# KKKSQJ/DeepLearning

Measured on NVIDIA H100. Metric: images/sec (ResNet-50 training step), higher is better.
Workload: dtype bf16

## Files before the change

### deeplearning_b200/csrc/abi_conv.cu

```cuda
#include <string.h>
#include "../../include/b200cls.h"
#include "conv_gemm.cuh"
#include "conv1x1_stream.cuh"
#include "conv_tap64.cuh"
#include "host_utils.h"
#include "wgrad_gemm.cuh"

using namespace b200;

namespace {

constexpr uint32_t kFwdDescLbo = 16, kFwdDescSbo = 1024;
constexpr uint32_t kWgDescLbo = 8192, kWgDescSbo = 1024, kWgDescKstep = 2048;

struct Box3 {
  int b1, b2, b3;
};

Box3 choose_box(long long d1, long long d2, long long d3, int P) {
  Box3 best{P, 1, 1};
  double best_cost = -1;
  for (int b1 = 1; b1 <= P; b1 <<= 1) {
    for (int b2 = 1; b1 * b2 <= P; b2 <<= 1) {
      const int b3 = P / (b1 * b2);
      if (b1 > 256 || b2 > 256 || b3 > 256) continue;
      const double c1 = double((d1 + b1 - 1) / b1) * b1, c2 = double((d2 + b2 - 1) / b2) * b2,
                   c3 = double((d3 + b3 - 1) / b3) * b3;
      const double cost = c1 * c2 * c3;
      if (best_cost < 0 || cost < best_cost - 0.5 ||
          (cost < best_cost + 0.5 && (b1 > best.b1 || (b1 == best.b1 && b2 > best.b2)))) {
        best_cost = cost;
        best = Box3{b1, b2, b3};
      }
    }
  }
  return best;
}
// ... 186 lines not shown
  if (p.residual) f |= p.res_f32 ? kEpiResF32 : kEpiResBf16;
  if (p.has_aux_out) f |= kEpiAux;
  if (p.out_f32) f |= kEpiOutF32;
  if (p.out_direct) f |= kEpiDirect;
  if (p.stats) f |= kEpiStats;
  if (p.rowscale) f |= kEpiRowscale;
  if (p.affine) f = (f & ~(kEpiBias | kEpiColscale)) | kEpiAffine;
  if (p.mask_in) f |= p.bn_scale ? kEpiBnMask : kEpiMask;
  if (p.bn_scale) f &= ~kEpiStats;
  return f;
}

#define B200_EPI_LIST(X)                                                                                  \
  X(kEpiStats)                                              \
  X(0)                                                      \
  X(kEpiResBf16)                                            \
  X(kEpiBias)                                               \
  X(kEpiBias | kEpiResF32 | kEpiOutF32)                     \
  X(kEpiBias | kEpiColscale | kEpiResF32 | kEpiOutF32)      \
  X(kEpiBias | (2 << kEpiActShift) | kEpiAux)               \
  X(3 << kEpiActShift)                                      \
  X((3 << kEpiActShift) | kEpiStats)                        \
  X(kEpiOutF32)                                             \
  X(kEpiBias | kEpiOutF32)                                  \
  X(kEpiAffine | kEpiResBf16 | (1 << kEpiActShift))        \
  X(kEpiAffine | (1 << kEpiActShift))                      \
  X(kEpiAffine)                                            \
  X(kEpiMask | kEpiResBf16 | kEpiStats)                    \
  X(kEpiBnMask)                                            \
  X(kEpiBnMask | kEpiBias)                                 \
  X(kEpiBias | (1 << kEpiActShift))                        \
  X(kEpiBias | kEpiStats)

bool tap64_ok(const ConvGemmParams& p) {
  const int f = epilogue_flags(p);
  return p.N == 64 && p.n_tiles == 1 && p.k_per_tap == 64 && p.k_blocks_per_tap == 1 && !p.var_taps && !p.chan_window &&
         p.num_taps >= 2 && p.num_taps <= 9 && (f == 0 || f == kEpiStats) && p.dim1 % p.box1 == 0 && p.dim2 % p.box2 == 0 &&
         p.dim3 % p.box3 == 0;
}
template <bool kStats>
int launch_tap64(const ConvGemmParams& q, int grid, cudaStream_t st) {
  static bool configured = false;
  if (!configured) {
    B200_CHECK_CUDA(cudaFuncSetAttribute(conv_tap64_kernel<kStats>, cudaFuncAttributeMaxDynamicSharedMemorySize, kTap64SmemBytes));
    configured = true;
  }
  B200_CHECK_CUDA(launch_pdl(conv_tap64_kernel<kStats>, dim3(grid), dim3(384), kTap64SmemBytes, st, q));
  B200_LAUNCHED();
  return OK;
}

template <int BLOCK_N>
int launch_conv_gemm(const ConvGemmParams& p, cudaStream_t st) {
  const int tiles = p.tiles1 * p.tiles2 * p.tiles3 * p.n_tiles;
  const int grid = conv_grid(tiles, p.n_tiles, p.stats != nullptr);
  B200_REQUIRE(grid > 0, "conv_gemm: %d channel blocks exceed the SM count (BN statistics need grid %% n_tiles == 0)", p.n_tiles);
  ConvGemmParams q = p;
  q.desc_lbo = kFwdDescLbo;
  q.desc_sbo = kFwdDescSbo;
  if constexpr (BLOCK_N == 64) {
    if (tap64_ok(p)) return p.stats != nullptr ? launch_tap64<true>(q, grid, st) : launch_tap64<false>(q, grid, st);
  }
  switch (epilogue_flags(p)) {
#define B200_EPI_CASE(F) \
  case (F):              \
    return launch_conv_gemm_epi<BLOCK_N, (F)>(q, grid, st);
    B200_EPI_LIST(B200_EPI_CASE)
#undef B200_EPI_CASE
    default:
      return launch_conv_gemm_epi<BLOCK_N, kEpiGeneric>(q, grid, st);
  }
}


bool stream_ok(long long pixels, int K, int N) {
  return (K == 64 || K == 128 || K == 256) && N % 256 == 0 && pixels % 128 == 0 && pixels / 128 < (1LL << 30);
}
int stream_grid(long long pixels, int N) {
  const int n_tiles = N / 256;
  const long long items = pixels / 128 * n_tiles;
  int grid = items < device_sm_count() ? static_cast<int>(items) : device_sm_count();
  return grid / n_tiles * n_tiles;
}

template <int KB, int MODE>
int launch_stream(const StreamParams& q, int grid, cudaStream_t st) {
  using Cfg = StreamCfg<KB, MODE>;
  static bool configured = false;
  if (!configured) {
    B200_CHECK_CUDA(cudaFuncSetAttribute(conv1x1_stream_kernel<KB, MODE>, cudaFuncAttributeMaxDynamicSharedMemorySize,
                                         Cfg::SMEM_BYTES));
    configured = true;
  }
  B200_CHECK_CUDA(launch_pdl(conv1x1_stream_kernel<KB, MODE>, dim3(grid), dim3(Cfg::THREADS), Cfg::SMEM_BYTES, st, q));
// ... 211 lines not shown
  B200_REQUIRE(bn_scale == nullptr || (Cout % 64 == 0 && bias == nullptr && stats == nullptr && out_f32 == nullptr && act <= 1 && !y_f32),
               "conv2d_fwd + folded BN: Cout=%d must be a multiple of 64, no bias / statistics / fp32 output", Cout);
  cudaStream_t st = static_cast<cudaStream_t>(stream);
  const int Ho = out_dim(H, ksize, stride), Wo = out_dim(W, ksize, stride);
  ConvGemmParams p;
  memset(&p, 0, sizeof(p));
  int rc;
  View dv = act_view(y, B, Ho, Wo, Cout, ksize == 1 && stride == 1);
  if (out_f32 != nullptr) dv.base = nullptr;
  if ((rc = setup_output(p, dv, Cout, y_f32, nullptr))) return rc;
  const int BN = Cg ? 64 : block_n_for(Cout);
  p.n_tiles = (Cout + BN - 1) / BN;
  p.chan_window = Cg ? 1 : 0;
  p.k_per_tap = Cg ? 64 : Cin;
  p.k_blocks_per_tap = Cg ? 1 : (Cin + 63) / 64;
  p.num_taps = ksize * ksize;
  if ((rc = encode_taps(p, p.a_maps, x, B, H, W, Cin, ksize, stride, box_of(p)))) return rc;
  for (int t = 0; t < p.num_taps; ++t) p.tap_w[t] = static_cast<int8_t>(t);
  if ((rc = encode_matrix(&p.b_map, w, static_cast<long long>(p.num_taps) * p.k_per_tap, Cout, BN))) return rc;
  p.stats = stats;
  p.bias = bias;
  p.act = act;
  p.residual = residual;
  p.rs1 = static_cast<long long>(dv.strides[1]);
  p.rs2 = static_cast<long long>(dv.strides[2]);
  p.rs3 = static_cast<long long>(dv.strides[3]);
  p.out_direct = out_f32;
  p.ld_out = ld_out;
  if (bn_scale != nullptr) {
    p.affine = 1;
    p.colscale = bn_scale;
    p.bias = bn_shift;
  }
  return Cg ? launch_conv_gemm<64>(p, st) : dispatch_conv_gemm(p, Cout, st);
}

int b200_conv2d_fwd(const void* x, const void* w, void* y, int B, int H, int W, int Cin, int Cout, int ksize, int stride,
                    float* stats, const float* bias, int act, const void* residual, float* out_f32, long long ld_out,
                    const float* bn_scale, const float* bn_shift, void* stream) {
  return conv_fwd(x, w, y, B, H, W, Cin, Cout, ksize, stride, stats, bias, act, residual, out_f32, ld_out, bn_scale, bn_shift,
                  0, 0, stream);
}

int b200_conv2d_fwd_f32(const void* x, const void* w, float* y, int B, int H, int W, int Cin, int Cout, int ksize,
                        int stride, const float* bias, void* stream) {
  return conv_fwd(x, w, y, B, H, W, Cin, Cout, ksize, stride, nullptr, bias, 0, nullptr, nullptr, 0, nullptr, nullptr, 1, 0,
                  stream);
}

static int conv_dgrad(const void* dy, const void* wd, void* dx, int B, int H, int W, int Cin, int Cout, int ksize,
                      int stride, const void* residual, const b200_bn_mask_t* bn_mask, int Cg, void* stream) {
  B200_REQUIRE(ksize == 1 || ksize == 3 || (ksize == 2 && stride == 2), "conv2d_dgrad: ksize %d / stride %d unsupported", ksize, stride);
  B200_REQUIRE(stride == 1 || stride == 2, "conv2d_dgrad: stride %d unsupported", stride);
  B200_REQUIRE(Cin % 8 == 0 && Cout % 8 == 0, "conv2d_dgrad: Cin=%d / Cout=%d must be multiples of 8", Cin, Cout);
  B200_REQUIRE(bn_mask == nullptr || (stride == 1 && Cin % 64 == 0 && bn_mask_complete(bn_mask)),
               "conv2d_dgrad: the fused BatchNorm-backward reduce needs stride 1, Cin %% 64 == 0 and every bn_mask field "
               "(Cin=%d, stride=%d)", Cin, stride);
  cudaStream_t st = static_cast<cudaStream_t>(stream);
  const int Ho = out_dim(H, ksize, stride), Wo = out_dim(W, ksize, stride);
  const bool flat = (ksize == 1 && stride == 1);
  const int BN = Cg ? 64 : block_n_for(Cin);
  const int k_per_tap = Cg ? 64 : Cout;
  int rc;
  CUtensorMap b_map;
  if ((rc = encode_matrix(&b_map, wd, static_cast<long long>(ksize * ksize) * k_per_tap, Cin, BN))) return rc;
  const int nphase = (stride == 2 && ksize >= 2) ? 2 : 1;
// ... 19 lines not shown
        for (int kh = 0; kh < 3; ++kh)
          for (int kw = 0; kw < 3; ++kw) {
            p.tap_map[nt] = 0;
            p.tap_o1[nt] = static_cast<int8_t>(1 - kw);
            p.tap_o2[nt] = static_cast<int8_t>(1 - kh);
            p.tap_w[nt] = static_cast<int8_t>(kh * 3 + kw);
            ++nt;
          }
      } else if (ksize == 2) {
        p.tap_map[0] = 0, p.tap_o1[0] = 0, p.tap_o2[0] = 0;
        p.tap_w[0] = static_cast<int8_t>(ph * 2 + pw);
        nt = 1;
      } else {
        for (int kh = 0; kh < 3; ++kh) {
          if (((ph + 1 - kh) & 1) != 0) continue;
          for (int kw = 0; kw < 3; ++kw) {
            if (((pw + 1 - kw) & 1) != 0) continue;
            p.tap_map[nt] = 0;
            p.tap_o1[nt] = static_cast<int8_t>((pw + 1 - kw) / 2);
            p.tap_o2[nt] = static_cast<int8_t>((ph + 1 - kh) / 2);
            p.tap_w[nt] = static_cast<int8_t>(kh * 3 + kw);
            ++nt;
          }
        }
      }
      p.num_taps = nt;
      if (residual != nullptr) {
        p.residual = static_cast<const char*>(residual) + (static_cast<const char*>(dv.base) - static_cast<const char*>(dx));
        p.rs1 = static_cast<long long>(dv.strides[1]);
        p.rs2 = static_cast<long long>(dv.strides[2]);
        p.rs3 = static_cast<long long>(dv.strides[3]);
      }
      if (bn_mask != nullptr) set_bn_mask(p, bn_mask, dv);
      if ((rc = Cg ? launch_conv_gemm<64>(p, st) : dispatch_conv_gemm(p, Cin, st))) return rc;
    }
  }
  return OK;
}

int b200_conv2d_dgrad(const void* dy, const void* wd, void* dx, int B, int H, int W, int Cin, int Cout, int ksize,
                      int stride, const void* residual, const b200_bn_mask_t* bn_mask, void* stream) {
  return conv_dgrad(dy, wd, dx, B, H, W, Cin, Cout, ksize, stride, residual, bn_mask, 0, stream);
}

int b200_gemm_ex(const b200_view_t* a, const b200_view_t* out, const b200_gemm_args_t* g, void* stream) {
  B200_REQUIRE(a != nullptr && out != nullptr && g != nullptr && g->w != nullptr, "gemm_ex: null argument");
  B200_REQUIRE(g->N % 8 == 0 && g->K % 8 == 0, "gemm_ex: N=%d / K=%d must be multiples of 8", g->N, g->K);
  for (int i = 0; i < 3; ++i)
    B200_REQUIRE(a->dim[i] == out->dim[i] && a->dim[i] > 0, "gemm_ex: a/out pixel extents differ in dim %d", i);
  B200_REQUIRE(!(g->aux_out != nullptr && g->out_f32), "gemm_ex: aux_out needs a bf16 primary output");
  B200_REQUIRE(!(g->stats != nullptr && g->out_f32), "gemm_ex: stats need a bf16 output");
  auto to_view = [](const b200_view_t* v, int C) {
    View r;
    r.base = v->base;
    r.dims[0] = C;
    r.strides[0] = 1;
    for (int i = 0; i < 3; ++i) {
      r.dims[i + 1] = static_cast<uint64_t>(v->dim[i]);
      r.strides[i + 1] = static_cast<uint64_t>(v->stride[i]);
    }
    return r;
  };
  ConvGemmParams p;
  memset(&p, 0, sizeof(p));
  int rc;
  View dv = to_view(out, g->N);
// ... 56 lines not shown
  if (pl.block_ng == 64)
    rc = launch_wgrad<64>(p, st);
  else if (pl.block_ng == 128)
    rc = launch_wgrad<128>(p, st);
  else if (pl.block_ng == 192)
    rc = launch_wgrad<192>(p, st);
  else
    rc = launch_wgrad<256>(p, st);
  if (rc) return rc;
  if ((rc = launch_wgrad_reduce(p.partial, dw, pl.splits, Cout, Cin, pl.taps, accumulate, st, bias_partial, bias_out))) return rc;
  B200_LAUNCHED();
  return OK;
}

int b200_stem_s2d_conv_fwd(const void* z, const void* w, void* y, float* stats, int B, int Ho, int Wo, void* stream) {
  B200_REQUIRE(B > 0 && Ho > 0 && Wo > 0, "stem_s2d_conv_fwd: empty output");
  cudaStream_t st = static_cast<cudaStream_t>(stream);
  const int Cout = 64;
  ConvGemmParams p;
  memset(&p, 0, sizeof(p));
  int rc;
  if ((rc = setup_output(p, make_view(y, B, Ho, Wo, Cout, 1, 0, 0), Cout, 0, nullptr))) return rc;
  const Box3 bx = box_of(p);
  p.k_per_tap = 64;
  p.k_blocks_per_tap = 1;
  p.num_taps = 4;
  if ((rc = encode_view(&p.a_maps[0], stem_s2d_view(z, B, Ho, Wo), bx))) return rc;
  for (int i = 1; i < 4; ++i) p.a_maps[i] = p.a_maps[0];
  for (int ky = 0; ky < 4; ++ky) {
    p.tap_map[ky] = 0, p.tap_o1[ky] = 0, p.tap_o2[ky] = static_cast<int8_t>(ky), p.tap_w[ky] = static_cast<int8_t>(ky);
  }
  if ((rc = encode_matrix(&p.b_map, w, 256, Cout, 64))) return rc;
  p.stats = stats;
  return dispatch_conv_gemm(p, Cout, st);
}

size_t b200_stem_s2d_conv_wgrad_workspace_bytes(int B, int Ho, int Wo) {
  return wgrad_bytes(plan_wgrad_geom(Wo, Ho, B, 64, 64, 4), 64, 64);
}

int b200_stem_s2d_conv_wgrad(const void* dy, const void* z, float* g, void* workspace, size_t workspace_bytes, int B, int Ho,
                             int Wo, void* stream) {
  cudaStream_t st = static_cast<cudaStream_t>(stream);
  const int Cout = 64, Cin = 64, taps = 4;
  const WgradPlan pl = plan_wgrad_geom(Wo, Ho, B, Cin, Cout, taps);
  const size_t need = wgrad_bytes(pl, Cout, Cin);
  B200_REQUIRE(workspace != nullptr && workspace_bytes >= need, "stem_s2d_conv_wgrad: workspace too small (%zu < %zu)",
               workspace_bytes, need);
  WgradParams p = wgrad_params(pl, Cout, Cin, workspace);
  int rc;
  if ((rc = encode_view(&p.dy_map, make_view(dy, B, Ho, Wo, Cout, 1, 0, 0), pl.box))) return rc;
  if ((rc = encode_view(&p.x_maps[0], stem_s2d_view(z, B, Ho, Wo), pl.box))) return rc;
  for (int i = 1; i < 4; ++i) p.x_maps[i] = p.x_maps[0];
  for (int ky = 0; ky < 4; ++ky) p.tap_map[ky] = 0, p.tap_o1[ky] = 0, p.tap_o2[ky] = static_cast<int8_t>(ky);
  if ((rc = launch_wgrad<256>(p, st))) return rc;
  if ((rc = launch_wgrad_reduce(p.partial, g, pl.splits, Cout, Cin, taps, 0, st))) return rc;
  B200_LAUNCHED();
  return OK;
}


int b200_conv1x1_bn_act_fwd(const void* x, const void* w, const float* scale, const float* shift, const void* residual,
                            void* y, long long pixels, int Cin, int Cout, int relu, void* stream) {
  B200_REQUIRE(pixels > 0 && Cin % 64 == 0 && Cout % 64 == 0, "conv1x1_bn_act_fwd: Cin=%d / Cout=%d must be multiples of 64", Cin, Cout);
  B200_REQUIRE(scale != nullptr && shift != nullptr && residual != nullptr && relu == 1,
               "conv1x1_bn_act_fwd: implemented for relu(bn(conv) + residual)");
// ... 162 lines not shown
```

### deeplearning_b200/csrc/conv_gemm.cuh

```cuda
#pragma once
#include <cstdio>
#include "common.cuh"

namespace b200 {

constexpr int kMaxTaps = 16;

struct alignas(64) ConvGemmParams {
  CUtensorMap a_maps[4];
  CUtensorMap b_map;
  CUtensorMap d_map;
  CUtensorMap aux_map;
  int num_taps;
  int k_per_tap;
  int k_blocks_per_tap;
  int tiles1, tiles2, tiles3;
  int box1, box2, box3;
  int dim1, dim2, dim3;
  int qoff1[4], qoff2[4], qoff3[4];
  int n_tiles;
  int N;
  int8_t tap_map[kMaxTaps];
  int8_t tap_o1[kMaxTaps];
  int8_t tap_o2[kMaxTaps];
  int8_t tap_w[kMaxTaps];
  float* stats;
  const float* bias;
  const float* colscale;
  int act;
  int out_f32;
  int res_f32;
  int has_aux_out;
  const void* residual;
  long long rs1, rs2, rs3;
  const __nv_bfloat16* aux_in;
  long long as1, as2, as3;
  uint32_t desc_lbo, desc_sbo;
  float* out_direct;
  long long ld_out;
  const float* rowscale;
  int rows_per_sample;
  int var_taps;
  int kb_total;
  int16_t tap_kb[kMaxTaps];
  int32_t tap_k0[kMaxTaps];
  const __nv_bfloat16* mask_in;
  long long ms1, ms2, ms3;
  int affine;
  const float* bn_scale;
  const float* bn_shift;
  int chan_window;
};

template <int BLOCK_N>
struct ConvGemmCfg {
  static constexpr int BLOCK_M = 128;
  static constexpr int BLOCK_K = 64;
  static constexpr int A_BYTES = BLOCK_M * BLOCK_K * 2;
  static constexpr int B_BYTES = BLOCK_N * BLOCK_K * 2;
  static constexpr int STAGES = BLOCK_N == 128 ? 4 : 5;
  static constexpr int STAGE_BYTES = A_BYTES + B_BYTES;
  static constexpr int EPI_WARPS = 4;
  static constexpr int SLAB_BYTES = 32 * 128;
  static constexpr int STAGING_BYTES = EPI_WARPS * 2 * SLAB_BYTES;
  static constexpr int IMG_BYTES = BLOCK_M * BLOCK_N * 4;
  static constexpr int IMGS = BLOCK_N == 128 ? 1 : 2;
  static constexpr int BAR_BYTES = 256;
  static constexpr int SMEM_BYTES = STAGES * STAGE_BYTES + STAGING_BYTES + IMGS * IMG_BYTES + BAR_BYTES + 1024;
  static constexpr int THREADS = 512;
  static_assert(SMEM_BYTES <= 227 * 1024, "shared memory of one H100 block");
  static_assert(2 * STAGES + 2 * IMGS <= BAR_BYTES / 8, "mbarriers");
};

__device__ __forceinline__ void gelu_parts(float x, float& tail, float& e) {
  const float az = fabsf(x) * 0.70710678118654752f;
  float t;
  asm("rcp.approx.ftz.f32 %0, %1;" : "=f"(t) : "f"(fmaf(0.3275911f, az, 1.0f)));
  float poly = fmaf(1.061405429f, t, -1.453152027f);
  poly = fmaf(poly, t, 1.421413741f);
  poly = fmaf(poly, t, -0.284496736f);
  poly = fmaf(poly, t, 0.254829592f);
  asm("ex2.approx.ftz.f32 %0, %1;" : "=f"(e) : "f"(-1.4426950408889634f * az * az));
  tail = 0.5f * poly * t * e;
}
__device__ __forceinline__ float gelu_erf(float x) {
  float tail, e;
  gelu_parts(x, tail, e);
  return x * (x >= 0.f ? 1.0f - tail : tail);
}
__device__ __forceinline__ float gelu_erf_grad(float x) {
  float tail, e;
  gelu_parts(x, tail, e);
  const float cdf = x >= 0.f ? 1.0f - tail : tail;
  return fmaf(x * 0.3989422804014327f, e, cdf);
}

__device__ __forceinline__ void gelu_parts2(float x0, float x1, uint64_t& cdf, uint64_t& e) {
  const uint64_t az = f2_pack(fabsf(x0) * 0.70710678118654752f, fabsf(x1) * 0.70710678118654752f);
  float d0, d1, t0, t1, g0, g1, e0, e1, h0, h1;
  f2_unpack(f2_fma(f2_bcast(0.3275911f), az, f2_bcast(1.0f)), d0, d1);
  asm("rcp.approx.ftz.f32 %0, %1;" : "=f"(t0) : "f"(d0));
  asm("rcp.approx.ftz.f32 %0, %1;" : "=f"(t1) : "f"(d1));
  const uint64_t t = f2_pack(t0, t1);
  uint64_t poly = f2_fma(f2_bcast(1.061405429f), t, f2_bcast(-1.453152027f));
// ... 15 lines not shown
__device__ __forceinline__ void gelu_erf_val_grad2(float& x0, float& x1, float& g0, float& g1) {
  uint64_t cdf, e;
  gelu_parts2(x0, x1, cdf, e);
  const uint64_t x = f2_pack(x0, x1);
  f2_unpack(f2_fma(f2_mul(x, f2_bcast(0.3989422804014327f)), e, cdf), g0, g1);
  f2_unpack(f2_mul(x, cdf), x0, x1);
}

#ifdef CONV_PROFILE
#define CPROF_DECL(N) long long cp_t[N] = {}; long long cp_0 = clock64(), cp_1;
#define CPROF_TICK(i) { cp_1 = clock64(); cp_t[i] += cp_1 - cp_0; cp_0 = cp_1; }
#else
#define CPROF_DECL(N)
#define CPROF_TICK(i)
#endif

template <int S>
__device__ __forceinline__ void butterfly_step(float (&px)[32], int lane) {
  const bool up = (lane & S) != 0;
#pragma unroll
  for (int i = 0; i < S; ++i) {
    const float send = up ? px[i] : px[i + S];
    const float keep = up ? px[i + S] : px[i];
    px[i] = keep + __shfl_xor_sync(0xffffffffu, send, S);
  }
}

constexpr int kEpiGeneric = -1;
constexpr int kEpiBias = 1, kEpiColscale = 2, kEpiActShift = 2 , kEpiResBf16 = 16, kEpiResF32 = 32,
              kEpiAux = 64, kEpiOutF32 = 128, kEpiDirect = 256, kEpiStats = 512,
              kEpiRowscale = 1024 ,
              kEpiAffine = 2048, kEpiMask = 4096, kEpiBnMask = 8192;

template <int BLOCK_N, int EPI = kEpiGeneric>
__global__ void __launch_bounds__(512, 1) conv_gemm_kernel(const __grid_constant__ ConvGemmParams p) {
  static_assert(BLOCK_N == 64 || BLOCK_N == 128, "64- or 128-column tiles");
  using Cfg = ConvGemmCfg<BLOCK_N>;
  constexpr int STAGES = Cfg::STAGES;
  constexpr int IMGS = Cfg::IMGS;
  extern __shared__ uint8_t smem_raw[];
  uint8_t* smem = reinterpret_cast<uint8_t*>((reinterpret_cast<uintptr_t>(smem_raw) + 1023) & ~uintptr_t(1023));
  uint8_t* stage_base = smem;
  uint8_t* staging = smem + STAGES * Cfg::STAGE_BYTES;
  uint8_t* img = staging + Cfg::STAGING_BYTES;
  uint64_t* bars = reinterpret_cast<uint64_t*>(img + IMGS * Cfg::IMG_BYTES);
  uint64_t* full_bar = bars;
  uint64_t* empty_bar = bars + STAGES;
  uint64_t* img_full = bars + 2 * STAGES;
  uint64_t* img_empty = bars + 2 * STAGES + IMGS;

  const int warp_idx = threadIdx.x >> 5;
  const int lane = threadIdx.x & 31;
  const int m_tiles = p.tiles1 * p.tiles2 * p.tiles3;
  const int num_tiles = m_tiles * p.n_tiles;
  const int num_kb = p.var_taps ? p.kb_total : p.num_taps * p.k_blocks_per_tap;

  if (warp_idx == 0 && lane == 0) {
    for (int i = 0; i < 4; ++i) tma_prefetch_desc(&p.a_maps[i]);
    tma_prefetch_desc(&p.b_map);
    tma_prefetch_desc(&p.d_map);
    for (int i = 0; i < STAGES; ++i) {
      mbar_init(&full_bar[i], 1);
      mbar_init(&empty_bar[i], 2);
    }
    for (int i = 0; i < IMGS; ++i) {
      mbar_init(&img_full[i], 8);
      mbar_init(&img_empty[i], Cfg::EPI_WARPS);
    }
    fence_mbar_init();
  }
  __syncthreads();
  pdl_wait();

  if (warp_idx < 4) {
    setmaxnreg_dec<40>();
    if (warp_idx == 0 && lane == 0) {
      int stage = 0;
      uint32_t phase = 0;
      CPROF_DECL(2)
      for (int tile = blockIdx.x; tile < num_tiles; tile += gridDim.x) {
        const int n_tile = tile % p.n_tiles;
        const int m_tile = tile / p.n_tiles;
        const int t1 = m_tile % p.tiles1;
        const int t2 = (m_tile / p.tiles1) % p.tiles2;
        const int t3 = m_tile / (p.tiles1 * p.tiles2);
        const int c1 = t1 * p.box1, c2 = t2 * p.box2, c3 = t3 * p.box3;
        int tap = 0, cb = 0;
        int kb_in_tap = p.var_taps ? p.tap_kb[0] : p.k_blocks_per_tap;
        for (int kb = 0; kb < num_kb; ++kb, ++cb) {
          if (cb == kb_in_tap) {
            cb = 0;
            ++tap;
            if (p.var_taps) kb_in_tap = p.tap_kb[tap];
          }
          const int wk = p.var_taps ? p.tap_k0[tap] + cb * 64 : p.tap_w[tap] * p.k_per_tap + cb * 64;
          CPROF_TICK(1)
          mbar_wait_backoff(&empty_bar[stage], phase ^ 1);
          CPROF_TICK(0)
          uint8_t* a_dst = stage_base + stage * Cfg::STAGE_BYTES;
          uint8_t* b_dst = a_dst + Cfg::A_BYTES;
          mbar_expect_tx(&full_bar[stage], Cfg::STAGE_BYTES);
          tma_load_4d(a_dst, &p.a_maps[p.tap_map[tap]], &full_bar[stage], p.chan_window ? n_tile * BLOCK_N : cb * 64, c1 + p.tap_o1[tap],
                      c2 + p.tap_o2[tap], c3);
          tma_load_2d(b_dst, &p.b_map, &full_bar[stage], wk, n_tile * BLOCK_N);
          if (++stage == STAGES) {
            stage = 0;
            phase ^= 1;
          }
        }
      }
#ifdef CONV_PROFILE
      if (blockIdx.x == 0) {
        const int nt = (num_tiles - 1) / gridDim.x + 1;
        printf("conv producer: wait_empty %lld issue %lld  (cycles/tile, %d tiles, %d k-blocks)\n", cp_t[0] / nt, cp_t[1] / nt, nt, num_kb);
      }
#endif
    }
  } else if (warp_idx < 12) {
    setmaxnreg_dec<112>();
    const int wg = (warp_idx - 4) >> 2;
    const uint64_t desc_a0 = make_smem_desc_sw128(smem_u32(stage_base) + wg * 8192, p.desc_lbo, p.desc_sbo);
    const uint64_t desc_b0 = make_smem_desc_sw128(smem_u32(stage_base) + Cfg::A_BYTES, p.desc_lbo, p.desc_sbo);
    int stage = 0;
    uint32_t phase = 0;
    int it = 0;
    CPROF_DECL(3)
    for (int tile = blockIdx.x; tile < num_tiles; tile += gridDim.x, ++it) {
      float acc[BLOCK_N / 2];
#pragma unroll
      for (int i = 0; i < BLOCK_N / 2; ++i) acc[i] = 0.f;
      int prev = -1;
      CPROF_TICK(2)
      for (int kb = 0; kb < num_kb; ++kb) {
        mbar_wait(&full_bar[stage], phase);
        wgmma_fence();
        const uint64_t soff = static_cast<uint64_t>(stage) * (Cfg::STAGE_BYTES >> 4);
        const uint64_t da = desc_a0 + soff, db = desc_b0 + soff;
#pragma unroll
        for (int k = 0; k < 4; ++k) Wgmma<BLOCK_N, 0, 0>::mma(acc, da + 2 * k, db + 2 * k, 1u);
        wgmma_commit();
        wgmma_wait<1>();
        if (prev >= 0 && (threadIdx.x & 127) == 0) mbar_arrive(&empty_bar[prev]);
        prev = stage;
        if (++stage == STAGES) {
          stage = 0;
          phase ^= 1;
        }
      }
      wgmma_wait<0>();
      wgmma_reg_fence(acc);
      if ((threadIdx.x & 127) == 0) mbar_arrive(&empty_bar[prev]);
      CPROF_TICK(0)
      const int b = IMGS == 1 ? 0 : it % IMGS;
      mbar_wait(&img_empty[b], ((it / IMGS) & 1) ^ 1);
      CPROF_TICK(1)
      acc_to_img<BLOCK_N>(acc, smem_u32(img + b * Cfg::IMG_BYTES), BLOCK_N, 64 * wg, 0);
      __syncwarp();
      if (lane == 0) mbar_arrive(&img_full[b]);
    }
#ifdef CONV_PROFILE
    if (blockIdx.x == 0 && lane == 0 && (warp_idx & 3) == 0) {
      const int nt = (num_tiles - 1) / gridDim.x + 1;
      printf("conv mma wg %d: main loop %lld wait img_empty %lld acc->img %lld  (cycles/tile)\n", wg, cp_t[0] / nt, cp_t[1] / nt,
             cp_t[2] / nt);
    }
#endif
  } else {
    setmaxnreg_inc<248>();
    const int q = warp_idx - 12;
    const int row = q * 32 + lane;
    const uint32_t stage_s = smem_u32(staging + q * 2 * Cfg::SLAB_BYTES);
    const uint32_t row_s = lane * 128;
    const uint32_t sw = (lane & 7) << 4;
    uint32_t stat_off[8];
#pragma unroll
    for (int m = 0; m < 8; ++m) stat_off[m] = m * 128 + ((((lane >> 2) ^ m) << 4) | ((lane & 3) << 2));
    constexpr bool G = EPI < 0;
    constexpr bool kAffine = !G && (EPI & kEpiAffine) != 0;
    constexpr bool kBnMask = !G && (EPI & kEpiBnMask) != 0;
    constexpr bool kMask = !G && (EPI & (kEpiMask | kEpiBnMask)) != 0;
    const int N = p.N;
    const float* const bias = (!kAffine && (G || (EPI & kEpiBias))) ? p.bias : nullptr;
    const float* const colscale = (!kAffine && (G || (EPI & kEpiColscale))) ? p.colscale : nullptr;
    const int act_bits = G ? p.act : ((EPI >> kEpiActShift) & 3);
    const int act = kAffine ? 0 : act_bits;
    const bool has_res = G ? (p.residual != nullptr) : ((EPI & (kEpiResBf16 | kEpiResF32)) != 0);
    const bool res_f32 = G ? (p.res_f32 != 0) : ((EPI & kEpiResF32) != 0);
    const bool has_aux = G ? (p.has_aux_out != 0) : ((EPI & kEpiAux) != 0);
    const bool out_f32 = G ? (p.out_f32 != 0) : ((EPI & kEpiOutF32) != 0);
    float* const out_direct = (G || (EPI & kEpiDirect)) ? p.out_direct : nullptr;
    float* const stats = (G || (EPI & (kEpiStats | kEpiBnMask))) ? p.stats : nullptr;
    const float* const rowscale = G ? p.rowscale : nullptr;
    const bool need_rowmap = has_res || act == 3 || kMask || out_direct != nullptr || rowscale != nullptr || p.dim1 % p.box1 != 0 ||
                             p.dim2 % p.box2 != 0 || p.dim3 % p.box3 != 0;
    const bool full_cols = (N % BLOCK_N) == 0;
    uint32_t store_counter = 0;
    const int unit_cols = out_f32 ? 32 : 64;
    const int units = BLOCK_N / unit_cols;
    const int nsub = out_f32 ? 1 : 2;
    constexpr int SLOTS = 2;
    uint64_t run_s[SLOTS], run_q[SLOTS];
    float run_x[SLOTS][2];
#pragma unroll
    for (int k = 0; k < SLOTS; ++k) run_s[k] = 0, run_q[k] = 0, run_x[k][0] = run_x[k][1] = 0.f;
// ... 31 lines not shown
            const float4* rp = reinterpret_cast<const float4*>(static_cast<const float*>(p.residual) + off);
#pragma unroll
            for (int j = 0; j < 8; ++j)
              if (full_cols || ncp + j * 4 < N) nx_f[j] = __ldg(rp + j);
          } else {
            const uint4* rp = reinterpret_cast<const uint4*>(static_cast<const __nv_bfloat16*>(p.residual) + off);
#pragma unroll
            for (int j = 0; j < 4; ++j)
              if (full_cols || ncp + j * 8 < N) nx_b[j] = __ldg(rp + j);
          }
        }
        if (act == 3) {
          const uint4* ap = reinterpret_cast<const uint4*>(p.aux_in + p3 * p.as3 + p2 * p.as2 + p1 * p.as1 + ncp);
#pragma unroll
          for (int j = 0; j < 4; ++j)
            if (full_cols || ncp + j * 8 < N) nx_b[j] = __ldg(ap + j);
        }
        if constexpr (kMask) {
          const uint4* mp = reinterpret_cast<const uint4*>(p.mask_in + p3 * p.ms3 + p2 * p.ms2 + p1 * p.ms1 + ncp);
#pragma unroll
          for (int j = 0; j < 4; ++j)
            if (full_cols || ncp + j * 8 < N) nx_m[j] = __ldg(mp + j);
        }
      };
      if (has_res || act == 3 || kMask) issue_pre(0, 0);
      CPROF_TICK(1)
      mbar_wait(&img_full[b], (it / IMGS) & 1);
      CPROF_TICK(0)

#pragma unroll 1
      for (int u = 0; u < units; ++u) {
        const int n0 = n_tile * BLOCK_N + u * unit_cols;
        const bool chunk_live = n0 < N;
        const uint32_t buf_s = stage_s + (store_counter & 1) * Cfg::SLAB_BYTES;
        const uint32_t aux_s = stage_s + ((store_counter + 1) & 1) * Cfg::SLAB_BYTES;
        if (chunk_live && out_direct == nullptr) {
          if (lane == 0) {
            if (has_aux) tma_store_wait_read<0>(); else tma_store_wait_read<1>();
          }
          __syncwarp();
        }
#pragma unroll 1
        for (int h = 0; h < nsub; ++h) {
          uint32_t v[32];
          img_ld32(img_s, BLOCK_N, row, u * unit_cols + h * 32, v);
          if (u == units - 1 && h == nsub - 1) {
            __syncwarp();
            if (lane == 0) mbar_arrive(&img_empty[b]);
          }
          uint4 pre_b[4];
          float4 pre_f[8];
          uint4 pre_m[4];
          if (has_res || act == 3 || kMask) {
#pragma unroll
            for (int j = 0; j < 4; ++j) pre_b[j] = nx_b[j];
#pragma unroll
            for (int j = 0; j < 8; ++j) pre_f[j] = nx_f[j];
            if constexpr (kMask) {
#pragma unroll
              for (int j = 0; j < 4; ++j) pre_m[j] = nx_m[j];
            }
            if (h + 1 < nsub)
              issue_pre(u, h + 1);
            else if (u + 1 < units)
              issue_pre(u + 1, 0);
          }
          if (!chunk_live) continue;
          const int nc = n0 + h * 32;
          float f[32];
#pragma unroll
          for (int j = 0; j < 32; ++j) f[j] = __uint_as_float(v[j]);
// ... 257 lines not shown
```

### deeplearning_b200/csrc/conv_tap64.cuh

```cuda
#pragma once
#include "conv_gemm.cuh"

namespace b200 {

constexpr int kTap64Stages = 5;
constexpr int kTap64SmemBytes = 9 * 8192 + kTap64Stages * 16384 + 8 * 4096 + 128 * 64 * 4 + 512 + 1024;
static_assert(kTap64SmemBytes <= 227 * 1024, "shared memory of one H100 block");

template <bool kStats>
__global__ void __launch_bounds__(384, 1) conv_tap64_kernel(const __grid_constant__ ConvGemmParams p) {
  constexpr int STAGES = kTap64Stages;
  extern __shared__ uint8_t smem_raw[];
  uint8_t* smem = reinterpret_cast<uint8_t*>((reinterpret_cast<uintptr_t>(smem_raw) + 1023) & ~uintptr_t(1023));
  uint8_t* sB = smem;
  uint8_t* sA = sB + 9 * 8192;
  uint8_t* sOut = sA + STAGES * 16384;
  uint8_t* sImg = sOut + 8 * 4096;
  uint64_t* bars = reinterpret_cast<uint64_t*>(sImg + 128 * 64 * 4);
  uint64_t* a_full = bars;
  uint64_t* a_empty = bars + STAGES;
  uint64_t* b_full = bars + 2 * STAGES;

  const int warp_idx = threadIdx.x >> 5, lane = threadIdx.x & 31;
  const int m_tiles = p.tiles1 * p.tiles2 * p.tiles3;
  const int taps = p.num_taps;

  if (warp_idx == 0 && lane == 0) {
    for (int i = 0; i < 4; ++i) tma_prefetch_desc(&p.a_maps[i]);
    tma_prefetch_desc(&p.b_map);
    tma_prefetch_desc(&p.d_map);
    for (int i = 0; i < STAGES; ++i) {
      mbar_init(&a_full[i], 1);
      mbar_init(&a_empty[i], 2);
    }
    mbar_init(b_full, 1);
    fence_mbar_init();
  }
  __syncthreads();
  pdl_wait();

  if (warp_idx < 4) {
    setmaxnreg_dec<40>();
    if (warp_idx == 0 && lane == 0) {
      mbar_expect_tx(b_full, static_cast<uint32_t>(taps) * 8192u);
      for (int t = 0; t < taps; ++t) tma_load_2d(sB + t * 8192, &p.b_map, b_full, p.tap_w[t] * p.k_per_tap, 0);
      int stage = 0;
      uint32_t phase = 0;
      for (int tile = blockIdx.x; tile < m_tiles; tile += gridDim.x) {
        const int t1 = tile % p.tiles1;
        const int t2 = (tile / p.tiles1) % p.tiles2;
        const int t3 = tile / (p.tiles1 * p.tiles2);
        const int c1 = t1 * p.box1, c2 = t2 * p.box2, c3 = t3 * p.box3;
        for (int t = 0; t < taps; ++t) {
          mbar_wait_backoff(&a_empty[stage], phase ^ 1);
          mbar_expect_tx(&a_full[stage], 16384);
          tma_load_4d(sA + stage * 16384, &p.a_maps[p.tap_map[t]], &a_full[stage], 0, c1 + p.tap_o1[t], c2 + p.tap_o2[t], c3);
          if (++stage == STAGES) {
            stage = 0;
            phase ^= 1;
          }
        }
      }
    }
  } else {
    setmaxnreg_inc<232>();
    const int ew = warp_idx - 4;
    const int wg = ew >> 2;
    const int q = 2 * wg + (ew & 1);
    const int pair = (ew >> 1) & 1;
    const int row = q * 32 + lane;
    const uint32_t img_s = smem_u32(sImg);
    const uint64_t desc_a0 = make_smem_desc_sw128(smem_u32(sA) + wg * 8192, p.desc_lbo, p.desc_sbo);
    const uint64_t desc_b0 = make_smem_desc_sw128(smem_u32(sB), p.desc_lbo, p.desc_sbo);
    const uint32_t os = smem_u32(sOut + ew * 4096);
    const uint32_t row_s = lane * 128;
    const uint32_t sw = (lane & 7) << 4;
    uint32_t stat_off[8];
#pragma unroll
    for (int m = 0; m < 8; ++m) stat_off[m] = m * 128 + ((((lane >> 2) ^ m) << 4) | ((lane & 3) << 2));
    uint64_t run_s = 0, run_q = 0;
    mbar_wait(b_full, 0);
    int stage = 0;
    uint32_t phase = 0;
    int it = 0;
    for (int tile = blockIdx.x; tile < m_tiles; tile += gridDim.x, ++it) {
      float acc[32];
#pragma unroll
      for (int i = 0; i < 32; ++i) acc[i] = 0.f;
      int prev = -1;
      for (int t = 0; t < taps; ++t) {
        mbar_wait(&a_full[stage], phase);
        wgmma_fence();
        const uint64_t da = desc_a0 + static_cast<uint64_t>(stage) * (16384 >> 4);
        const uint64_t db = desc_b0 + static_cast<uint64_t>(t) * (8192 >> 4);
#pragma unroll
        for (int k = 0; k < 4; ++k) Wgmma<64, 0, 0>::mma(acc, da + 2 * k, db + 2 * k, 1u);
        wgmma_commit();
        wgmma_wait<1>();
        if (prev >= 0 && (threadIdx.x & 127) == 0) mbar_arrive(&a_empty[prev]);
        prev = stage;
        if (++stage == STAGES) {
          stage = 0;
          phase ^= 1;
        }
      }
      wgmma_wait<0>();
      wgmma_reg_fence(acc);
      if ((threadIdx.x & 127) == 0) mbar_arrive(&a_empty[prev]);
      named_bar_sync(1 + wg, 128);
      acc_to_img<64>(acc, img_s, 64, 64 * wg, 0);
      named_bar_sync(1 + wg, 128);
      if ((it & 1) != pair) continue;
      const int t1 = tile % p.tiles1;
      const int t2 = (tile / p.tiles1) % p.tiles2;
      const int t3 = tile / (p.tiles1 * p.tiles2);
      const int s1 = t1 * p.box1 + p.qoff1[q], s2 = t2 * p.box2 + p.qoff2[q], s3 = t3 * p.box3 + p.qoff3[q];
      if (lane == 0) tma_store_wait_read<0>();
      __syncwarp();
#pragma unroll
      for (int h = 0; h < 2; ++h) {
        uint32_t v[32];
        img_ld32(img_s, 64, row, h * 32, v);
#pragma unroll
        for (int j = 0; j < 4; ++j)
          sts128(os + row_s + (((h * 4 + j) << 4) ^ sw),
                 pack_bf16x2(__uint_as_float(v[j * 8 + 0]), __uint_as_float(v[j * 8 + 1])),
                 pack_bf16x2(__uint_as_float(v[j * 8 + 2]), __uint_as_float(v[j * 8 + 3])),
                 pack_bf16x2(__uint_as_float(v[j * 8 + 4]), __uint_as_float(v[j * 8 + 5])),
                 pack_bf16x2(__uint_as_float(v[j * 8 + 6]), __uint_as_float(v[j * 8 + 7])));
      }
      __syncwarp();
      if constexpr (kStats) {
        uint64_t a_s = 0, a_q = 0;
#pragma unroll
        for (int r = 0; r < 32; ++r) {
          const uint32_t w = lds32(os + (r >> 3) * 1024 + stat_off[r & 7]);
          const uint64_t x2 = f2_pack(bf16_lo(w), bf16_hi(w));
          a_s = f2_add(a_s, x2);
          a_q = f2_fma(x2, x2, a_q);
        }
        run_s = f2_add(run_s, a_s);
        run_q = f2_add(run_q, a_q);
      }
      fence_proxy_async_smem();
      __syncwarp();
      if (lane == 0) {
        asm volatile("cp.async.bulk.tensor.4d.global.shared::cta.bulk_group [%0, {%2, %3, %4, %5}], [%1];" ::"l"(
                         reinterpret_cast<uint64_t>(&p.d_map)),
                     "r"(os), "r"(0), "r"(s1), "r"(s2), "r"(s3)
                     : "memory");
        tma_store_commit();
      }
    }
    if constexpr (kStats) {
      const long long srow = (static_cast<long long>(blockIdx.x) * 4 + q) * 2 + pair;
      float s_lo, s_hi, q_lo, q_hi;
      f2_unpack(run_s, s_lo, s_hi);
      f2_unpack(run_q, q_lo, q_hi);
      float* sp = p.stats + srow * 2 * p.N + 2 * lane;
      *reinterpret_cast<float2*>(sp) = make_float2(s_lo, s_hi);
      *reinterpret_cast<float2*>(sp + p.N) = make_float2(q_lo, q_hi);
    }
    if (lane == 0) tma_store_wait_all<0>();
  }
}

}
```

Baseline: 8688.

## Replace tap64 kernel with halo A-feed path in conv_gemm kernel

Removes the dedicated tap64 kernel, which issued one TMA load per tap per tile. In its place, a HALO template variant of conv_gemm_kernel loads one halo slab per distinct column offset and shares it across taps, addressing each tap by a row offset into the slab. This cuts A-operand global/TMA traffic for 3x3 stride-1 convs with 64 output channels. The path also extends to the BN-mask epilogue, dgrad and the stem. In exchange it uses single-buffered epilogue staging, more complex slot/phase bookkeeping, and a different epilogue (the generic conv_gemm one rather than the custom paired-store one).

```diff
diff --git a/deeplearning_b200/csrc/abi_conv.cu b/deeplearning_b200/csrc/abi_conv.cu
--- a/deeplearning_b200/csrc/abi_conv.cu
+++ b/deeplearning_b200/csrc/abi_conv.cu
@@ -2,7 +2,6 @@
 #include "../../include/b200cls.h"
 #include "conv_gemm.cuh"
 #include "conv1x1_stream.cuh"
-#include "conv_tap64.cuh"
 #include "host_utils.h"
 #include "wgrad_gemm.cuh"
 
@@ -255,20 +254,58 @@
   X(kEpiBias | (1 << kEpiActShift))                        \
   X(kEpiBias | kEpiStats)
 
-bool tap64_ok(const ConvGemmParams& p) {
+int setup_halo(ConvGemmParams& p, const View& a) {
+  using Cfg = ConvGemmCfg<64>;
   const int f = epilogue_flags(p);
-  return p.N == 64 && p.n_tiles == 1 && p.k_per_tap == 64 && p.k_blocks_per_tap == 1 && !p.var_taps && !p.chan_window &&
-         p.num_taps >= 2 && p.num_taps <= 9 && (f == 0 || f == kEpiStats) && p.dim1 % p.box1 == 0 && p.dim2 % p.box2 == 0 &&
-         p.dim3 % p.box3 == 0;
-}
-template <bool kStats>
-int launch_tap64(const ConvGemmParams& q, int grid, cudaStream_t st) {
+  if (!(p.N == 64 && p.n_tiles == 1 && p.k_per_tap == 64 && p.k_blocks_per_tap == 1 && !p.var_taps && !p.chan_window &&
+        p.num_taps >= 2 && p.num_taps <= 9 && (f == 0 || f == kEpiStats || f == kEpiBnMask) && p.box1 % 8 == 0 &&
+        (p.box3 == 2 || (p.box3 == 1 && 64 % p.box1 == 0)) && p.dim1 % p.box1 == 0 && p.dim2 % p.box2 == 0 &&
+        p.dim3 % p.box3 == 0))
+    return OK;
+  int lo = p.tap_o2[0], hi = p.tap_o2[0], slabs = 0;
+  int8_t slab_o1[kMaxTaps], tap_slab[kMaxTaps];
+  for (int t = 0; t < p.num_taps; ++t) {
+    if (p.tap_map[t] != 0) return OK;
+    lo = p.tap_o2[t] < lo ? p.tap_o2[t] : lo;
+    hi = p.tap_o2[t] > hi ? p.tap_o2[t] : hi;
+    int s = 0;
+    while (s < slabs && slab_o1[s] != p.tap_o1[t]) ++s;
+    if (s == slabs) slab_o1[slabs++] = p.tap_o1[t];
+    tap_slab[t] = static_cast<int8_t>(s);
+  }
+  const int rows2 = p.box2 + hi - lo;
+  const int bytes = p.box1 * rows2 * p.box3 * 128;
+  const int stride = (bytes + 1023) / 1024 * 1024;
+  if (slabs > Cfg::HALO_SLOTS || p.num_taps * 8192 + Cfg::HALO_SLOTS * stride > Cfg::HALO_AB_BYTES || rows2 > 256) return OK;
+  int rc;
+  if ((rc = encode_view(&p.a_maps[0], a, Box3{p.box1, rows2, p.box3}))) return rc;
+  p.halo_slabs = slabs;
+  p.halo_bytes = bytes;
+  p.halo_stride = stride;
+  p.halo_o2 = lo;
+  p.halo_wg_rows = p.box3 == 1 ? 64 : p.box1 * rows2;
+  for (int s = 0; s < slabs; ++s) p.slab_o1[s] = slab_o1[s];
+  p.halo_last = 0;
+  for (int t = 0; t < p.num_taps; ++t) {
+    p.tap_slab[t] = tap_slab[t];
+    p.tap_row[t] = static_cast<int16_t>(p.box1 * (p.tap_o2[t] - lo));
+    bool later = false;
+    for (int u = t + 1; u < p.num_taps; ++u) later |= tap_slab[u] == tap_slab[t];
+    if (!later) p.halo_last |= 1u << t;
+  }
+  return OK;
+}
+
+template <int EPI>
+int launch_halo(const ConvGemmParams& q, int grid, cudaStream_t st) {
+  using Cfg = ConvGemmCfg<64>;
   static bool configured = false;
   if (!configured) {
-    B200_CHECK_CUDA(cudaFuncSetAttribute(conv_tap64_kernel<kStats>, cudaFuncAttributeMaxDynamicSharedMemorySize, kTap64SmemBytes));
+    B200_CHECK_CUDA(cudaFuncSetAttribute(conv_gemm_kernel<64, EPI, true>, cudaFuncAttributeMaxDynamicSharedMemorySize,
+                                         Cfg::HALO_SMEM_BYTES));
     configured = true;
   }
-  B200_CHECK_CUDA(launch_pdl(conv_tap64_kernel<kStats>, dim3(grid), dim3(384), kTap64SmemBytes, st, q));
+  B200_CHECK_CUDA(launch_pdl(conv_gemm_kernel<64, EPI, true>, dim3(grid), dim3(Cfg::THREADS), Cfg::HALO_SMEM_BYTES, st, q));
   B200_LAUNCHED();
   return OK;
 }
@@ -282,7 +319,11 @@
   q.desc_lbo = kFwdDescLbo;
   q.desc_sbo = kFwdDescSbo;
   if constexpr (BLOCK_N == 64) {
-    if (tap64_ok(p)) return p.stats != nullptr ? launch_tap64<true>(q, grid, st) : launch_tap64<false>(q, grid, st);
+    if (p.halo_slabs > 0) {
+      const int f = epilogue_flags(p);
+      return f == kEpiStats ? launch_halo<kEpiStats>(q, grid, st)
+                            : (f == kEpiBnMask ? launch_halo<kEpiBnMask>(q, grid, st) : launch_halo<0>(q, grid, st));
+    }
   }
   switch (epilogue_flags(p)) {
 #define B200_EPI_CASE(F) \
@@ -560,6 +601,7 @@
     p.colscale = bn_scale;
     p.bias = bn_shift;
   }
+  if (stride == 1 && !Cg && (rc = setup_halo(p, act_view(x, B, H, W, Cin, ksize == 1)))) return rc;
   return Cg ? launch_conv_gemm<64>(p, st) : dispatch_conv_gemm(p, Cout, st);
 }
 
@@ -645,6 +687,7 @@
         p.rs3 = static_cast<long long>(dv.strides[3]);
       }
       if (bn_mask != nullptr) set_bn_mask(p, bn_mask, dv);
+      if (stride == 1 && !Cg && (rc = setup_halo(p, act_view(dy, B, Ho, Wo, Cout, flat)))) return rc;
       if ((rc = Cg ? launch_conv_gemm<64>(p, st) : dispatch_conv_gemm(p, Cin, st))) return rc;
     }
   }
@@ -767,6 +810,7 @@
   }
   if ((rc = encode_matrix(&p.b_map, w, 256, Cout, 64))) return rc;
   p.stats = stats;
+  if ((rc = setup_halo(p, stem_s2d_view(z, B, Ho, Wo)))) return rc;
   return dispatch_conv_gemm(p, Cout, st);
 }
 
diff --git a/deeplearning_b200/csrc/conv_gemm.cuh b/deeplearning_b200/csrc/conv_gemm.cuh
--- a/deeplearning_b200/csrc/conv_gemm.cuh
+++ b/deeplearning_b200/csrc/conv_gemm.cuh
@@ -50,6 +50,15 @@
   const float* bn_scale;
   const float* bn_shift;
   int chan_window;
+  int halo_slabs;
+  int halo_bytes;
+  int halo_stride;
+  int halo_o2;
+  int halo_wg_rows;
+  uint32_t halo_last;
+  int8_t slab_o1[kMaxTaps];
+  int8_t tap_slab[kMaxTaps];
+  int16_t tap_row[kMaxTaps];
 };
 
 template <int BLOCK_N>
@@ -70,6 +79,12 @@
   static constexpr int THREADS = 512;
   static_assert(SMEM_BYTES <= 227 * 1024, "shared memory of one H100 block");
   static_assert(2 * STAGES + 2 * IMGS <= BAR_BYTES / 8, "mbarriers");
+  static constexpr int HALO_SLOTS = 5;
+  static constexpr int HALO_AB_BYTES = 9 * BLOCK_N * 128 + HALO_SLOTS * 8 * 10 * 2 * 128;
+  static constexpr int HALO_STAGING_BYTES = EPI_WARPS * SLAB_BYTES;
+  static constexpr int HALO_SMEM_BYTES = HALO_AB_BYTES + HALO_STAGING_BYTES + IMG_BYTES + BAR_BYTES + 1024;
+  static_assert(BLOCK_N == 128 || HALO_SMEM_BYTES <= 227 * 1024, "shared memory of one H100 block (halo A-feed)");
+  static_assert(2 * HALO_SLOTS + 2 + 1 <= BAR_BYTES / 8, "mbarriers (halo A-feed)");
 };
 
 __device__ __forceinline__ void gelu_parts(float x, float& tail, float& e) {
@@ -151,22 +166,25 @@
               kEpiRowscale = 1024 ,
               kEpiAffine = 2048, kEpiMask = 4096, kEpiBnMask = 8192;
 
-template <int BLOCK_N, int EPI = kEpiGeneric>
+template <int BLOCK_N, int EPI = kEpiGeneric, bool HALO = false>
 __global__ void __launch_bounds__(512, 1) conv_gemm_kernel(const __grid_constant__ ConvGemmParams p) {
   static_assert(BLOCK_N == 64 || BLOCK_N == 128, "64- or 128-column tiles");
+  static_assert(!HALO || BLOCK_N == 64, "halo A-feed: 64-column tiles");
   using Cfg = ConvGemmCfg<BLOCK_N>;
-  constexpr int STAGES = Cfg::STAGES;
-  constexpr int IMGS = Cfg::IMGS;
+  constexpr int STAGES = HALO ? Cfg::HALO_SLOTS : Cfg::STAGES;
+  constexpr int IMGS = HALO ? 1 : Cfg::IMGS;
   extern __shared__ uint8_t smem_raw[];
   uint8_t* smem = reinterpret_cast<uint8_t*>((reinterpret_cast<uintptr_t>(smem_raw) + 1023) & ~uintptr_t(1023));
-  uint8_t* stage_base = smem;
-  uint8_t* staging = smem + STAGES * Cfg::STAGE_BYTES;
-  uint8_t* img = staging + Cfg::STAGING_BYTES;
+  uint8_t* stage_base = HALO ? smem + p.num_taps * (BLOCK_N * 128) : smem;
+  uint8_t* staging = smem + (HALO ? Cfg::HALO_AB_BYTES : STAGES * Cfg::STAGE_BYTES);
+  constexpr int STAGING_BUFS = HALO ? 1 : 2;
+  uint8_t* img = staging + Cfg::EPI_WARPS * STAGING_BUFS * Cfg::SLAB_BYTES;
   uint64_t* bars = reinterpret_cast<uint64_t*>(img + IMGS * Cfg::IMG_BYTES);
   uint64_t* full_bar = bars;
   uint64_t* empty_bar = bars + STAGES;
   uint64_t* img_full = bars + 2 * STAGES;
   uint64_t* img_empty = bars + 2 * STAGES + IMGS;
+  uint64_t* w_full = bars + 2 * STAGES + 2 * IMGS;
 
   const int warp_idx = threadIdx.x >> 5;
   const int lane = threadIdx.x & 31;
@@ -186,6 +204,7 @@
       mbar_init(&img_full[i], 8);
       mbar_init(&img_empty[i], Cfg::EPI_WARPS);
     }
+    if (HALO) mbar_init(w_full, 1);
     fence_mbar_init();
   }
   __syncthreads();
@@ -193,7 +212,27 @@
 
   if (warp_idx < 4) {
     setmaxnreg_dec<40>();
-    if (warp_idx == 0 && lane == 0) {
+    if (HALO && warp_idx == 0 && lane == 0) {
+      mbar_expect_tx(w_full, static_cast<uint32_t>(p.num_taps) * (BLOCK_N * 128));
+      for (int t = 0; t < p.num_taps; ++t) tma_load_2d(smem + t * (BLOCK_N * 128), &p.b_map, w_full, p.tap_w[t] * p.k_per_tap, 0);
+      int slot = 0;
+      uint32_t phase = 0;
+      for (int tile = blockIdx.x; tile < num_tiles; tile += gridDim.x) {
+        const int t1 = tile % p.tiles1;
+        const int t2 = (tile / p.tiles1) % p.tiles2;
+        const int t3 = tile / (p.tiles1 * p.tiles2);
+        for (int s = 0; s < p.halo_slabs; ++s) {
+          mbar_wait_backoff(&empty_bar[slot], phase ^ 1);
+          mbar_expect_tx(&full_bar[slot], p.halo_bytes);
+          tma_load_4d(stage_base + slot * p.halo_stride, &p.a_maps[0], &full_bar[slot], 0, t1 * p.box1 + p.slab_o1[s],
+                      t2 * p.box2 + p.halo_o2, t3 * p.box3);
+          if (++slot == STAGES) {
+            slot = 0;
+            phase ^= 1;
+          }
+        }
+      }
+    } else if (warp_idx == 0 && lane == 0) {
       int stage = 0;
       uint32_t phase = 0;
       CPROF_DECL(2)
@@ -243,6 +282,10 @@
     int stage = 0;
     uint32_t phase = 0;
     int it = 0;
+    const uint64_t desc_w = make_smem_desc_sw128(smem_u32(smem), p.desc_lbo, p.desc_sbo);
+    const uint64_t desc_slab0 =
+        make_smem_desc_sw128(smem_u32(stage_base) + (HALO ? wg * p.halo_wg_rows * 128 : 0), p.desc_lbo, p.desc_sbo);
+    if (HALO) mbar_wait(w_full, 0);
     CPROF_DECL(3)
     for (int tile = blockIdx.x; tile < num_tiles; tile += gridDim.x, ++it) {
       float acc[BLOCK_N / 2];
@@ -250,7 +293,26 @@
       for (int i = 0; i < BLOCK_N / 2; ++i) acc[i] = 0.f;
       int prev = -1;
       CPROF_TICK(2)
-      for (int kb = 0; kb < num_kb; ++kb) {
+      if constexpr (HALO) {
+        for (int t = 0; t < p.num_taps; ++t) {
+          int slot = stage + p.tap_slab[t];
+          uint32_t ph = phase;
+          if (slot >= STAGES) slot -= STAGES, ph ^= 1;
+          mbar_wait(&full_bar[slot], ph);
+          wgmma_fence();
+          const uint64_t da = desc_slab0 + static_cast<uint64_t>((slot * p.halo_stride + p.tap_row[t] * 128) >> 4);
+          const uint64_t db = desc_w + static_cast<uint64_t>(t * (BLOCK_N * 128 >> 4));
+#pragma unroll
+          for (int k = 0; k < 4; ++k) Wgmma<BLOCK_N, 0, 0>::mma(acc, da + 2 * k, db + 2 * k, 1u);
+          wgmma_commit();
+          wgmma_wait<1>();
+          if (prev >= 0 && (threadIdx.x & 127) == 0) mbar_arrive(&empty_bar[prev]);
+          prev = (p.halo_last >> t) & 1u ? slot : -1;
+        }
+        stage += p.halo_slabs;
+        if (stage >= STAGES) stage -= STAGES, phase ^= 1;
+      }
+      for (int kb = 0; kb < (HALO ? 0 : num_kb); ++kb) {
         mbar_wait(&full_bar[stage], phase);
         wgmma_fence();
         const uint64_t soff = static_cast<uint64_t>(stage) * (Cfg::STAGE_BYTES >> 4);
@@ -268,7 +330,7 @@
       }
       wgmma_wait<0>();
       wgmma_reg_fence(acc);
-      if ((threadIdx.x & 127) == 0) mbar_arrive(&empty_bar[prev]);
+      if (prev >= 0 && (threadIdx.x & 127) == 0) mbar_arrive(&empty_bar[prev]);
       CPROF_TICK(0)
       const int b = IMGS == 1 ? 0 : it % IMGS;
       mbar_wait(&img_empty[b], ((it / IMGS) & 1) ^ 1);
@@ -288,7 +350,7 @@
     setmaxnreg_inc<248>();
     const int q = warp_idx - 12;
     const int row = q * 32 + lane;
-    const uint32_t stage_s = smem_u32(staging + q * 2 * Cfg::SLAB_BYTES);
+    const uint32_t stage_s = smem_u32(staging + q * STAGING_BUFS * Cfg::SLAB_BYTES);
     const uint32_t row_s = lane * 128;
     const uint32_t sw = (lane & 7) << 4;
     uint32_t stat_off[8];
@@ -386,11 +448,11 @@
       for (int u = 0; u < units; ++u) {
         const int n0 = n_tile * BLOCK_N + u * unit_cols;
         const bool chunk_live = n0 < N;
-        const uint32_t buf_s = stage_s + (store_counter & 1) * Cfg::SLAB_BYTES;
-        const uint32_t aux_s = stage_s + ((store_counter + 1) & 1) * Cfg::SLAB_BYTES;
+        const uint32_t buf_s = stage_s + (store_counter % STAGING_BUFS) * Cfg::SLAB_BYTES;
+        const uint32_t aux_s = stage_s + ((store_counter + 1) % STAGING_BUFS) * Cfg::SLAB_BYTES;
         if (chunk_live && out_direct == nullptr) {
           if (lane == 0) {
-            if (has_aux) tma_store_wait_read<0>(); else tma_store_wait_read<1>();
+            if (has_aux || STAGING_BUFS == 1) tma_store_wait_read<0>(); else tma_store_wait_read<1>();
           }
           __syncwarp();
         }
diff --git a/deeplearning_b200/csrc/conv_tap64.cuh b/deeplearning_b200/csrc/conv_tap64.cuh
--- a/deeplearning_b200/csrc/conv_tap64.cuh
+++ /dev/null
@@ -1,168 +0,0 @@
-#pragma once
-#include "conv_gemm.cuh"
-
-namespace b200 {
-
-constexpr int kTap64Stages = 5;
-constexpr int kTap64SmemBytes = 9 * 8192 + kTap64Stages * 16384 + 8 * 4096 + 128 * 64 * 4 + 512 + 1024;
-static_assert(kTap64SmemBytes <= 227 * 1024, "shared memory of one H100 block");
-
-template <bool kStats>
-__global__ void __launch_bounds__(384, 1) conv_tap64_kernel(const __grid_constant__ ConvGemmParams p) {
-  constexpr int STAGES = kTap64Stages;
-  extern __shared__ uint8_t smem_raw[];
-  uint8_t* smem = reinterpret_cast<uint8_t*>((reinterpret_cast<uintptr_t>(smem_raw) + 1023) & ~uintptr_t(1023));
-  uint8_t* sB = smem;
-  uint8_t* sA = sB + 9 * 8192;
-  uint8_t* sOut = sA + STAGES * 16384;
-  uint8_t* sImg = sOut + 8 * 4096;
-  uint64_t* bars = reinterpret_cast<uint64_t*>(sImg + 128 * 64 * 4);
-  uint64_t* a_full = bars;
-  uint64_t* a_empty = bars + STAGES;
-  uint64_t* b_full = bars + 2 * STAGES;
-
-  const int warp_idx = threadIdx.x >> 5, lane = threadIdx.x & 31;
-  const int m_tiles = p.tiles1 * p.tiles2 * p.tiles3;
-  const int taps = p.num_taps;
-
-  if (warp_idx == 0 && lane == 0) {
-    for (int i = 0; i < 4; ++i) tma_prefetch_desc(&p.a_maps[i]);
-    tma_prefetch_desc(&p.b_map);
-    tma_prefetch_desc(&p.d_map);
-    for (int i = 0; i < STAGES; ++i) {
-      mbar_init(&a_full[i], 1);
-      mbar_init(&a_empty[i], 2);
-    }
-    mbar_init(b_full, 1);
-    fence_mbar_init();
-  }
-  __syncthreads();
-  pdl_wait();
-
-  if (warp_idx < 4) {
-    setmaxnreg_dec<40>();
-    if (warp_idx == 0 && lane == 0) {
-      mbar_expect_tx(b_full, static_cast<uint32_t>(taps) * 8192u);
-      for (int t = 0; t < taps; ++t) tma_load_2d(sB + t * 8192, &p.b_map, b_full, p.tap_w[t] * p.k_per_tap, 0);
-      int stage = 0;
-      uint32_t phase = 0;
-      for (int tile = blockIdx.x; tile < m_tiles; tile += gridDim.x) {
-        const int t1 = tile % p.tiles1;
-        const int t2 = (tile / p.tiles1) % p.tiles2;
-        const int t3 = tile / (p.tiles1 * p.tiles2);
-        const int c1 = t1 * p.box1, c2 = t2 * p.box2, c3 = t3 * p.box3;
-        for (int t = 0; t < taps; ++t) {
-          mbar_wait_backoff(&a_empty[stage], phase ^ 1);
-          mbar_expect_tx(&a_full[stage], 16384);
-          tma_load_4d(sA + stage * 16384, &p.a_maps[p.tap_map[t]], &a_full[stage], 0, c1 + p.tap_o1[t], c2 + p.tap_o2[t], c3);
-          if (++stage == STAGES) {
-            stage = 0;
-            phase ^= 1;
-          }
-        }
-      }
-    }
-  } else {
-    setmaxnreg_inc<232>();
-    const int ew = warp_idx - 4;
-    const int wg = ew >> 2;
-    const int q = 2 * wg + (ew & 1);
-    const int pair = (ew >> 1) & 1;
-    const int row = q * 32 + lane;
-    const uint32_t img_s = smem_u32(sImg);
-    const uint64_t desc_a0 = make_smem_desc_sw128(smem_u32(sA) + wg * 8192, p.desc_lbo, p.desc_sbo);
-    const uint64_t desc_b0 = make_smem_desc_sw128(smem_u32(sB), p.desc_lbo, p.desc_sbo);
-    const uint32_t os = smem_u32(sOut + ew * 4096);
-    const uint32_t row_s = lane * 128;
-    const uint32_t sw = (lane & 7) << 4;
-    uint32_t stat_off[8];
-#pragma unroll
-    for (int m = 0; m < 8; ++m) stat_off[m] = m * 128 + ((((lane >> 2) ^ m) << 4) | ((lane & 3) << 2));
-    uint64_t run_s = 0, run_q = 0;
-    mbar_wait(b_full, 0);
-    int stage = 0;
-    uint32_t phase = 0;
-    int it = 0;
-    for (int tile = blockIdx.x; tile < m_tiles; tile += gridDim.x, ++it) {
-      float acc[32];
-#pragma unroll
-      for (int i = 0; i < 32; ++i) acc[i] = 0.f;
-      int prev = -1;
-      for (int t = 0; t < taps; ++t) {
-        mbar_wait(&a_full[stage], phase);
-        wgmma_fence();
-        const uint64_t da = desc_a0 + static_cast<uint64_t>(stage) * (16384 >> 4);
-        const uint64_t db = desc_b0 + static_cast<uint64_t>(t) * (8192 >> 4);
-#pragma unroll
-        for (int k = 0; k < 4; ++k) Wgmma<64, 0, 0>::mma(acc, da + 2 * k, db + 2 * k, 1u);
-        wgmma_commit();
-        wgmma_wait<1>();
-        if (prev >= 0 && (threadIdx.x & 127) == 0) mbar_arrive(&a_empty[prev]);
-        prev = stage;
-        if (++stage == STAGES) {
-          stage = 0;
-          phase ^= 1;
-        }
-      }
-      wgmma_wait<0>();
-      wgmma_reg_fence(acc);
-      if ((threadIdx.x & 127) == 0) mbar_arrive(&a_empty[prev]);
-      named_bar_sync(1 + wg, 128);
-      acc_to_img<64>(acc, img_s, 64, 64 * wg, 0);
-      named_bar_sync(1 + wg, 128);
-      if ((it & 1) != pair) continue;
-      const int t1 = tile % p.tiles1;
-      const int t2 = (tile / p.tiles1) % p.tiles2;
-      const int t3 = tile / (p.tiles1 * p.tiles2);
-      const int s1 = t1 * p.box1 + p.qoff1[q], s2 = t2 * p.box2 + p.qoff2[q], s3 = t3 * p.box3 + p.qoff3[q];
-      if (lane == 0) tma_store_wait_read<0>();
-      __syncwarp();
-#pragma unroll
-      for (int h = 0; h < 2; ++h) {
-        uint32_t v[32];
-        img_ld32(img_s, 64, row, h * 32, v);
-#pragma unroll
-        for (int j = 0; j < 4; ++j)
-          sts128(os + row_s + (((h * 4 + j) << 4) ^ sw),
-                 pack_bf16x2(__uint_as_float(v[j * 8 + 0]), __uint_as_float(v[j * 8 + 1])),
-                 pack_bf16x2(__uint_as_float(v[j * 8 + 2]), __uint_as_float(v[j * 8 + 3])),
-                 pack_bf16x2(__uint_as_float(v[j * 8 + 4]), __uint_as_float(v[j * 8 + 5])),
-                 pack_bf16x2(__uint_as_float(v[j * 8 + 6]), __uint_as_float(v[j * 8 + 7])));
-      }
-      __syncwarp();
-      if constexpr (kStats) {
-        uint64_t a_s = 0, a_q = 0;
-#pragma unroll
-        for (int r = 0; r < 32; ++r) {
-          const uint32_t w = lds32(os + (r >> 3) * 1024 + stat_off[r & 7]);
-          const uint64_t x2 = f2_pack(bf16_lo(w), bf16_hi(w));
-          a_s = f2_add(a_s, x2);
-          a_q = f2_fma(x2, x2, a_q);
-        }
-        run_s = f2_add(run_s, a_s);
-        run_q = f2_add(run_q, a_q);
-      }
-      fence_proxy_async_smem();
-      __syncwarp();
-      if (lane == 0) {
-        asm volatile("cp.async.bulk.tensor.4d.global.shared::cta.bulk_group [%0, {%2, %3, %4, %5}], [%1];" ::"l"(
-                         reinterpret_cast<uint64_t>(&p.d_map)),
-                     "r"(os), "r"(0), "r"(s1), "r"(s2), "r"(s3)
-                     : "memory");
-        tma_store_commit();
-      }
-    }
-    if constexpr (kStats) {
-      const long long srow = (static_cast<long long>(blockIdx.x) * 4 + q) * 2 + pair;
-      float s_lo, s_hi, q_lo, q_hi;
-      f2_unpack(run_s, s_lo, s_hi);
-      f2_unpack(run_q, q_lo, q_hi);
-      float* sp = p.stats + srow * 2 * p.N + 2 * lane;
-      *reinterpret_cast<float2*>(sp) = make_float2(s_lo, s_hi);
-      *reinterpret_cast<float2*>(sp + p.N) = make_float2(q_lo, q_hi);
-    }
-    if (lane == 0) tma_store_wait_all<0>();
-  }
-}
-
-}
```

After: 8757 (median of 6 runs). About the same (+0.8%).
